# NilFoundation/crypto3-zk

Measured on AMD Instinct MI355X. Metric: MSM Mpoints/sec, BLS12-381 G1 Pippenger, 2^20 points per GPU, higher is better.
Workload: dtype u32; 1 GPU; BLS12-381 G1 Pippenger MSM, ONE MSM of 1 x 2^20 random points/scalars, bases resident; points_per_gpu=1048576, parallelism=point-range partition x1 + one all-gather of the 144-B partial sums

## Files before the change

### crypto3-zk_amd/csrc/arith_ops.h

```cpp
#pragma once
#include "curve.hpp"
#include "fu_safegcd.hpp"

namespace zkhip {
namespace arith {

template <class U>
struct MaxSpread {
    static constexpr int K = 128;
};
template <>
struct MaxSpread<BlsFrU> {
    static constexpr int K = 64;
};
template <>
struct MaxSpread<PallasFrU> {
    static constexpr int K = 64;
};
template <>
struct MaxSpread<VestaFrU> {
    static constexpr int K = 64;
};

template <class U>
ZK_HD bool fu_raw_valid(int op) {
    if (op >= 0 && op <= 10) return true;
    return op >= 21 && op <= 27 && (1 << (op - 20)) <= MaxSpread<U>::K;
}

template <int K, class U>
ZK_HD Fu<U> sub_k(const Fu<U> &a, const Fu<U> &b) {
    if constexpr (K <= MaxSpread<U>::K) return fu_sub<K>(a, b);
    return Fu<U>::zero();
}

template <class U>
ZK_HD void fu_raw_one(int op, const uint32_t *a, const uint32_t *b, const uint32_t *c, const uint32_t *d, uint32_t *out) {
    constexpr int L = U::L;
    Fu<U> x, y, z, w, r = Fu<U>::zero();
    for (int i = 0; i < L; ++i) x.v[i] = a[i], y.v[i] = b[i], z.v[i] = c[i], w.v[i] = d[i];
    switch (op) {
        case 0: r = fu_mul(x, y); break;
        case 1: r = fu_sqr(x); break;
        case 2: r = fu_mul2(x, y, z, w); break;
        case 3: r = fu_add(x, y); break;
        case 4: r = fu_cond_sub_p(x); break;
        case 5: r = fu_canon(x); break;
        case 6: r.v[0] = fu_is_zero_lt2p(x) ? 1u : 0u; break;
        case 7: r = fu_inv(x); break;
        case 8: r = fu_inv_gcd(x); break;
        case 9: {
            uint32_t s[U::NL];
            fu_pack<U>(s, x);
            for (int i = 0; i < U::NL; ++i) r.v[i] = s[i];
            break;
        }
        case 10: r = fu_unpack<U>(a); break;
        case 21: r = sub_k<2>(x, y); break;
        case 22: r = sub_k<4>(x, y); break;
        case 23: r = sub_k<8>(x, y); break;
        case 24: r = sub_k<16>(x, y); break;
        case 25: r = sub_k<32>(x, y); break;
        case 26: r = sub_k<64>(x, y); break;
        case 27: r = sub_k<128>(x, y); break;
        default: break;
    }
    for (int i = 0; i < L; ++i) out[i] = r.v[i];
}

template <class F>
ZK_HD F sqr_direct(const F &x) { return FieldOps<F>::sqr(x); }
template <class U>
ZK_HD Fu<U> sqr_direct(const Fu<U> &x) { return fu_sqr(x); }

template <class F>
ZK_HD F inv_gcd(const F &x) { return FieldOps<F>::inv(x); }
template <class U>
ZK_HD Fu<U> inv_gcd(const Fu<U> &x) { return fu_inv_gcd(fu_canon(x)); }

ZK_HD bool field_op_valid(int op) { return op >= 0 && op <= 11; }

template <class F>
ZK_HD void field_op(int op, const uint32_t *a, const uint32_t *b, uint32_t *out) {
    typedef FieldOps<F> O;
    F x = O::from_canonical(a), y = b ? O::from_canonical(b) : F::zero(), r = F::zero();
    switch (op) {
        case 0: r = O::mul(x, y); break;
        case 1: r = O::add(x, y); break;
        case 2: r = O::template sub<O::K1>(x, y); break;
        case 3: r = O::inv(x); break;
// ... 1 lines not shown
        case 5: r = O::template sub<O::K1>(F::zero(), x); break;
        case 6: r = O::add(x, x); break;
        case 7: r = O::template sub<O::K2>(x, y); break;
        case 9: r = sqr_direct(O::add(x, y)); break;
        case 10: r = O::template mul_sub<O::K2>(x, O::add(x, y), O::template sub<O::K1>(F::zero(), y), y); break;
        case 11: r = inv_gcd(x); break;
        case 8: {
            F ab = O::mul(x, y), bb = O::sqr(y);
            F X = O::template sub<O::K1>(O::sqr(x), O::add(ab, O::add(bb, bb)));
            r = O::mul(O::template sub<O::K2>(ab, X), O::template sub<O::K2>(bb, X));
            break;
        }
        default: break;
    }
    O::to_canonical(out, r);
}

template <class F>
ZK_HD Affine<F> load_aff(const uint32_t *p, int inf) {
    typedef FieldOps<F> O;
    if (inf) return Affine<F>::infinity();
    return {O::from_canonical(p), O::from_canonical(p + O::CANON_WORDS)};
}
template <class F>
ZK_HD void store_aff(uint32_t *p, uint8_t *inf, const XYZZ<F> &a) {
    typedef FieldOps<F> O;
    Affine<F> r = xyzz_to_affine(a);
    *inf = a.is_inf() ? 1 : 0;
    O::to_canonical(p, r.x);
    O::to_canonical(p + O::CANON_WORDS, r.y);
}

template <class F>
ZK_HD void point_chain(const uint32_t *pts, const uint8_t *inf, const uint8_t *neg, size_t n, int mode, uint32_t k, uint32_t *out,
                       uint8_t *out_inf) {
    typedef FieldOps<F> O;
    constexpr int CW = O::CANON_WORDS;
    size_t split = mode == 1 ? n / 2 : n;
    XYZZ<F> acc = XYZZ<F>::infinity(), acc2 = XYZZ<F>::infinity();
    alignas(16) uint32_t b16[4 * O::WORDS];
    for (size_t i = 0; i < split; ++i) {
        Affine<F> p = load_aff<F>(pts + i * 2 * CW, inf ? inf[i] : 0);
        if (mode == 4) {
            affine_store<F>(b16, p);
            p = affine_load<F>(b16);
        }
        acc = xyzz_madd(acc, p, neg ? neg[i] != 0 : false);
        if (mode == 4) {
            xyzz_store<F>(b16, acc);
            acc = xyzz_load<F>(b16);
        }
    }
    for (size_t i = split; i < n; ++i) acc2 = xyzz_madd(acc2, load_aff<F>(pts + i * 2 * CW, inf ? inf[i] : 0), neg ? neg[i] != 0 : false);
    if (mode == 1) acc = xyzz_add(acc, acc2);
    if (mode == 2) acc = xyzz_mul_small(acc, k);
    if (mode == 3) {
        Jacobian<F> j = xyzz_to_jacobian(acc);
        O::to_canonical(out, j.X);
        O::to_canonical(out + CW, j.Y);
        O::to_canonical(out + 2 * CW, j.Z);
        *out_inf = acc.is_inf() ? 1 : 0;
        return;
    }
    store_aff<F>(out, out_inf, acc);
}

}
}
```

### crypto3-zk_amd/csrc/curve.hpp

```cpp
#pragma once
#include "fu.hpp"

namespace zkhip {

template <class F>
struct Affine {
    F x, y;
    ZK_HD bool is_inf() const { return FieldOps<F>::is_exact_zero(x) && FieldOps<F>::is_exact_zero(y); }
    ZK_HD static Affine infinity() { return {F::zero(), F::zero()}; }
};

template <class F>
struct XYZZ {
    F X, Y, ZZ, ZZZ;
    ZK_HD bool is_inf() const { return FieldOps<F>::is_exact_zero(ZZ); }
    ZK_HD static XYZZ infinity() { return {F::zero(), F::zero(), F::zero(), F::zero()}; }
    ZK_HD static XYZZ from_affine(const Affine<F> &p) {
        if (p.is_inf()) return infinity();
        return {p.x, p.y, F::one(), F::one()};
    }
};

template <class F>
struct Jacobian {
    F X, Y, Z;
};

template <class F>
ZK_HD XYZZ<F> xyzz_dbl_affine(const Affine<F> &p) {
    typedef FieldOps<F> O;
    if (p.is_inf()) return XYZZ<F>::infinity();
    F U = O::add(p.y, p.y);
    F V = O::sqr(U);
    F W = O::mul(U, V);
    F S = O::mul(p.x, V);
    F xx = O::sqr(p.x);
    F M = O::add(O::add(xx, xx), xx);
    F X3 = O::template sub<O::K1>(O::sqr(M), O::add(S, S));
    F Y3 = O::template mul_sub<O::K2>(M, O::template sub<O::K2>(S, X3), W, p.y);
    return {X3, Y3, V, W};
}

template <class F>
ZK_HD XYZZ<F> xyzz_dbl(const XYZZ<F> &a) {
    typedef FieldOps<F> O;
    if (a.is_inf()) return XYZZ<F>::infinity();
    F U = O::add(a.Y, a.Y);
    F V = O::sqr(U);
    F W = O::mul(U, V);
    F S = O::mul(a.X, V);
    F xx = O::sqr(a.X);
    F M = O::add(O::add(xx, xx), xx);
    F X3 = O::template sub<O::K1>(O::sqr(M), O::add(S, S));
    F Y3 = O::template mul_sub<O::K2>(M, O::template sub<O::K2>(S, X3), W, a.Y);
    return {X3, Y3, O::mul(V, a.ZZ), O::mul(W, a.ZZZ)};
}

template <class F>
ZK_HD XYZZ<F> xyzz_madd(const XYZZ<F> &a, const Affine<F> &p_in, bool negate = false) {
    typedef FieldOps<F> O;
    if (p_in.is_inf()) return a;
    Affine<F> p = p_in;
    if (negate) p.y = O::template sub<O::K1>(F::zero(), p.y);
    if (a.is_inf()) return {p.x, p.y, F::one(), F::one()};
    F U2 = O::mul(p.x, a.ZZ);
    F S2 = O::mul(p.y, a.ZZZ);
    F Pd = O::template sub<O::K2>(U2, a.X);
    F R = O::template sub<O::K2>(S2, a.Y);
    F PP = O::sqr(Pd);
    if (O::is_zero_product(PP)) {
        if (O::is_zero(R)) return xyzz_dbl_affine(p);
        return XYZZ<F>::infinity();
    }
    F PPP = O::mul(Pd, PP);
    F Q = O::mul(a.X, PP);
    F X3 = O::template sub<O::K1>(O::sqr(R), O::add(PPP, O::add(Q, Q)));
    F Y3 = O::template mul_sub<O::K2>(R, O::template sub<O::K2>(Q, X3), a.Y, PPP);
    return {X3, Y3, O::mul(a.ZZ, PP), O::mul(a.ZZZ, PPP)};
}

template <class F>
ZK_HD XYZZ<F> xyzz_add(const XYZZ<F> &a, const XYZZ<F> &b) {
    typedef FieldOps<F> O;
    if (a.is_inf()) return b;
    if (b.is_inf()) return a;
    F U1 = O::mul(a.X, b.ZZ);
    F U2 = O::mul(b.X, a.ZZ);
    F S1 = O::mul(a.Y, b.ZZZ);
    F S2 = O::mul(b.Y, a.ZZZ);
    F Pd = O::template sub<O::K1>(U2, U1);
    F R = O::template sub<O::K1>(S2, S1);
    F PP = O::sqr(Pd);
    if (O::is_zero_product(PP)) {
        if (O::is_zero(R)) return xyzz_dbl(a);
        return XYZZ<F>::infinity();
    }
    F PPP = O::mul(Pd, PP);
    F Q = O::mul(U1, PP);
    F X3 = O::template sub<O::K1>(O::sqr(R), O::add(PPP, O::add(Q, Q)));
    F Y3 = O::template mul_sub<O::K1>(R, O::template sub<O::K2>(Q, X3), S1, PPP);
    return {X3, Y3, O::mul(O::mul(a.ZZ, b.ZZ), PP), O::mul(O::mul(a.ZZZ, b.ZZZ), PPP)};
}

template <class F>
ZK_HD XYZZ<F> xyzz_mul_small(const XYZZ<F> &a, uint32_t k) {
    XYZZ<F> r = XYZZ<F>::infinity();
    if (k == 0 || a.is_inf()) return r;
    int top = 31;
    while (!((k >> top) & 1)) --top;
    if (top == 0) return a;
    const XYZZ<F> a2 = xyzz_dbl(a), a3 = xyzz_add(a2, a);
    for (int i = top >> 1; i >= 0; --i) {
        if (!r.is_inf()) r = xyzz_dbl(xyzz_dbl(r));
        const uint32_t d = (k >> (2 * i)) & 3u;
        if (d != 0) r = xyzz_add(r, d == 1 ? a : (d == 2 ? a2 : a3));
    }
    return r;
}

template <class F>
ZK_HD Jacobian<F> xyzz_to_jacobian(const XYZZ<F> &a) {
    typedef FieldOps<F> O;
    if (a.is_inf()) return {F::one(), F::one(), F::zero()};
    F z2 = O::sqr(a.ZZ);
    F z3 = O::sqr(a.ZZZ);
    return {O::mul(a.X, O::sqr(z2)), O::mul(a.Y, O::sqr(z3)), O::mul(a.ZZ, a.ZZZ)};
}

template <class F>
ZK_HD XYZZ<F> xyzz_from_jacobian(const Jacobian<F> &j) {
    typedef FieldOps<F> O;
    if (O::is_zero(j.Z)) return XYZZ<F>::infinity();
// ... 68 lines not shown
```

### crypto3-zk_amd/csrc/fu.hpp

```cpp
#pragma once
#include "fp.hpp"
#if defined(__HIP_DEVICE_COMPILE__) && !defined(ZK_NO_ASM_MUL)
#define ZK_ASM_MUL 1
#include "mont_asm.hpp"
#endif

namespace zkhip {

template <class U>
struct Fu {
    typedef U params;
    static constexpr int L = U::L;
    static constexpr int B = U::B;
    static constexpr int SL = U::SL;
    static constexpr uint32_t MASK = (1u << U::B) - 1;
    uint32_t v[L];

    ZK_HD static Fu zero() {
        Fu r;
ZK_UNROLL
        for (int i = 0; i < L; ++i) r.v[i] = 0;
        return r;
    }
    ZK_HD static Fu one() {
// ... 13 lines not shown
ZK_UNROLL
        for (int i = 0; i < L; ++i) r.v[i] = U::mod(i);
        return r;
    }
    ZK_HD bool limbs_zero() const {
        uint32_t o = 0;
ZK_UNROLL
        for (int i = 0; i < L; ++i) o |= v[i];
        return o == 0;
    }
    ZK_HD bool limbs_equal(const Fu &b) const {
        uint32_t o = 0;
ZK_UNROLL
        for (int i = 0; i < L; ++i) o |= v[i] ^ b.v[i];
        return o == 0;
    }
};

template <class U>
ZK_HD void fu_norm(Fu<U> &a) {
    constexpr int L = U::L, B = U::B;
ZK_UNROLL
    for (int i = 0; i < L - 1; ++i) {
        a.v[i + 1] += a.v[i] >> B;
        a.v[i] &= Fu<U>::MASK;
    }
}

template <class U>
ZK_HD Fu<U> fu_add(const Fu<U> &a, const Fu<U> &b) {
    Fu<U> r;
ZK_UNROLL
    for (int i = 0; i < U::L; ++i) r.v[i] = a.v[i] + b.v[i];
    fu_norm(r);
    return r;
}

template <int K, class U>
ZK_HD Fu<U> fu_sub(const Fu<U> &a, const Fu<U> &b) {
    Fu<U> r;
ZK_UNROLL
    for (int i = 0; i < U::L; ++i) r.v[i] = a.v[i] + (U::template spread<K>(i) - b.v[i]);
    fu_norm(r);
    return r;
}

template <class U>
ZK_HD Fu<U> fu_mul(const Fu<U> &a, const Fu<U> &b) {
    constexpr int L = U::L, B = U::B;
    constexpr uint32_t MASK = Fu<U>::MASK;
    Fu<U> r;
#ifdef ZK_ASM_MUL
    static_assert(B == 29, "mont_asm.hpp is generated for 29-bit limbs");
    uint32_t p[L];
ZK_UNROLL
    for (int i = 0; i < L; ++i) p[i] = U::mod(i);
    MontAsm<L>::mul(r.v, a.v, b.v, p, U::QINV);
    return r;
#endif
    uint32_t m[L];
    uint64_t acc = 0;
ZK_UNROLL
    for (int k = 0; k < L; ++k) {
ZK_UNROLL
        for (int i = 0; i <= k; ++i) acc += (uint64_t)a.v[i] * b.v[k - i];
ZK_UNROLL
// ... 209 lines not shown
        uint4 t;
        t.x = 4 * i + 0 < L ? a.v[4 * i + 0] : 0u;
        t.y = 4 * i + 1 < L ? a.v[4 * i + 1] : 0u;
        t.z = 4 * i + 2 < L ? a.v[4 * i + 2] : 0u;
        t.w = 4 * i + 3 < L ? a.v[4 * i + 3] : 0u;
        q[i] = t;
    }
}

template <class U>
struct Fu2 {
    typedef U params;
    Fu<U> c0, c1;
    ZK_HD static Fu2 zero() { return {Fu<U>::zero(), Fu<U>::zero()}; }
    ZK_HD static Fu2 one() { return {Fu<U>::one(), Fu<U>::zero()}; }
    ZK_HD bool limbs_zero() const { return c0.limbs_zero() && c1.limbs_zero(); }
};

template <class F>
struct FieldOps;

template <class P>
struct FieldOps<Fp<P>> {
    typedef Fp<P> F;
    static constexpr int K1 = 2, K2 = 2, K3 = 2;
    static constexpr int WORDS = P::NL;
    ZK_HD static F mul(const F &a, const F &b) { return a * b; }
    ZK_HD static F sqr(const F &a) { return a * a; }
    ZK_HD static F add(const F &a, const F &b) { return a + b; }
    template <int K>
    ZK_HD static F sub(const F &a, const F &b) { return a - b; }
    template <int K>
    ZK_HD static F mul_sub(const F &a, const F &b, const F &c, const F &d) { return mul(a, b) - mul(c, d); }
    ZK_HD static bool is_zero(const F &a) { return a.is_zero(); }
    ZK_HD static bool is_zero_product(const F &a) { return a.is_zero(); }
    ZK_HD static bool is_exact_zero(const F &a) { return a.is_zero(); }
    ZK_HD static F load(const uint32_t *p) { return fp_load<P>(p); }
    ZK_HD static void store(uint32_t *p, const F &a) { fp_store<P>(p, a); }
    ZK_HD static F from_canonical(const uint32_t *sat) { return fp_to_mont(fp_load<P>(sat)); }
    ZK_HD static void to_canonical(uint32_t *sat, const F &a) { fp_store<P>(sat, fp_from_mont(a)); }
    static constexpr int CANON_WORDS = P::NL;
    ZK_HD static F inv(const F &a) { return fp_inv(a); }
};

template <class P>
struct FieldOps<Fp2<P>> {
    typedef Fp2<P> F;
    static constexpr int K1 = 2, K2 = 2, K3 = 2;
    static constexpr int WORDS = 2 * P::NL;
    ZK_HD static F mul(const F &a, const F &b) { return a * b; }
    ZK_HD static F sqr(const F &a) { return fp_sqr(a); }
    ZK_HD static F add(const F &a, const F &b) { return a + b; }
    template <int K>
    ZK_HD static F sub(const F &a, const F &b) { return a - b; }
    template <int K>
    ZK_HD static F mul_sub(const F &a, const F &b, const F &c, const F &d) { return mul(a, b) - mul(c, d); }
    ZK_HD static bool is_zero(const F &a) { return a.is_zero(); }
    ZK_HD static bool is_zero_product(const F &a) { return a.is_zero(); }
    ZK_HD static bool is_exact_zero(const F &a) { return a.is_zero(); }
    ZK_HD static F load(const uint32_t *p) { return {fp_load<P>(p), fp_load<P>(p + P::NL)}; }
    ZK_HD static void store(uint32_t *p, const F &a) {
        fp_store<P>(p, a.c0);
        fp_store<P>(p + P::NL, a.c1);
    }
    ZK_HD static F from_canonical(const uint32_t *sat) { return {fp_to_mont(fp_load<P>(sat)), fp_to_mont(fp_load<P>(sat + P::NL))}; }
    ZK_HD static void to_canonical(uint32_t *sat, const F &a) {
        fp_store<P>(sat, fp_from_mont(a.c0));
        fp_store<P>(sat + P::NL, fp_from_mont(a.c1));
    }
    static constexpr int CANON_WORDS = 2 * P::NL;
    ZK_HD static F inv(const F &a) { return fp_inv(a); }
};

template <class U>
ZK_HD Fu<U> fu_mul_sel(const Fu<U> &a, const Fu<U> &b) {
#ifdef ZK_NOINLINE_MUL
    return fu_mul_call(a, b);
#else
    return fu_mul(a, b);
#endif
}

template <class U>
ZK_HD Fu<U> fu_mul_sel2(const Fu<U> &a, const Fu<U> &b) {
#if defined(ZK_NOINLINE_MUL) || defined(ZK_NOINLINE_MUL2)
    return fu_mul_call(a, b);
#else
    return fu_mul(a, b);
#endif
// ... 20 lines not shown
    }
    const Fu<U> a2 = fu_mul_call(a, a), a3 = fu_mul_call(a2, a);
    Fu<U> r = Fu<U>::one();
    for (int i = NL * 32 - 2; i >= 0; i -= 2) {
        r = fu_sqr_call(fu_sqr_call(r));
        const uint32_t w = (e[i >> 5] >> (i & 31)) & 3u;
        if (w == 1) r = fu_mul_call(r, a);
        else if (w == 2) r = fu_mul_call(r, a2);
        else if (w == 3) r = fu_mul_call(r, a3);
    }
    return r;
}

template <class U>
struct FieldOps<Fu<U>> {
    typedef Fu<U> F;
    static constexpr int K1 = 8, K2 = 16, K3 = 32;
    static constexpr int WORDS = U::SL;
    ZK_HD static F mul(const F &a, const F &b) { return fu_mul_sel(a, b); }
    ZK_HD static F sqr(const F &a) {
#ifdef ZK_NOINLINE_MUL
        return fu_mul_call(a, a);
#else
        return fu_sqr(a);
#endif
    }
    ZK_HD static F add(const F &a, const F &b) { return fu_add(a, b); }
    template <int K>
    ZK_HD static F sub(const F &a, const F &b) { return fu_sub<K>(a, b); }
    template <int K>
    ZK_HD static F mul_sub(const F &a, const F &b, const F &c, const F &d) {
        return fu_mul2_sel(a, b, fu_sub<K>(F::zero(), c), d);
    }
    ZK_HD static bool is_zero(const F &a) { return fu_canon(a).limbs_zero(); }
    ZK_HD static bool is_zero_product(const F &a) { return fu_is_zero_lt2p(a); }
    ZK_HD static bool is_exact_zero(const F &a) { return a.limbs_zero(); }
    ZK_HD static F load(const uint32_t *p) { return fu_load<U>(p); }
    ZK_HD static void store(uint32_t *p, const F &a) { fu_store<U>(p, a); }
    ZK_HD static F from_canonical(const uint32_t *sat) { return fu_from_canonical<U>(sat); }
    ZK_HD static void to_canonical(uint32_t *sat, const F &a) { fu_to_canonical<U>(sat, a); }
    static constexpr int CANON_WORDS = U::NL;
    ZK_HD static F inv(const F &a) { return fu_inv(a); }
};

template <class U>
struct FieldOps<Fu2<U>> {
    typedef Fu2<U> F;
    typedef FieldOps<Fu<U>> B;
    static constexpr int K1 = 32, K2 = 64, K3 = 128;
    static constexpr int WORDS = 2 * U::SL;
    ZK_HD static F mul(const F &a, const F &b) {
        Fu<U> v0 = fu_mul_sel2(a.c0, b.c0), v1 = fu_mul_sel2(a.c1, b.c1);
        Fu<U> s = fu_mul_sel2(fu_add(a.c0, a.c1), fu_add(b.c0, b.c1));
        return {fu_sub<4>(v0, v1), fu_sub<8>(s, fu_add(v0, v1))};
    }
    ZK_HD static F sqr(const F &a) {
        Fu<U> t = fu_mul_sel2(fu_add(a.c0, a.c1), fu_sub<128>(a.c0, a.c1));
        Fu<U> m = fu_mul_sel2(a.c0, a.c1);
        return {t, fu_add(m, m)};
    }
    ZK_HD static F add(const F &a, const F &b) { return {fu_add(a.c0, b.c0), fu_add(a.c1, b.c1)}; }
    template <int K>
    ZK_HD static F sub(const F &a, const F &b) { return {fu_sub<K>(a.c0, b.c0), fu_sub<K>(a.c1, b.c1)}; }
    template <int K>
    ZK_HD static F mul_sub(const F &a, const F &b, const F &c, const F &d) { return sub<K1>(mul(a, b), mul(c, d)); }
    ZK_HD static bool is_zero(const F &a) { return fu_canon(a.c0).limbs_zero() && fu_canon(a.c1).limbs_zero(); }
    ZK_HD static bool is_zero_product(const F &a) { return is_zero(a); }
    ZK_HD static bool is_exact_zero(const F &a) { return a.limbs_zero(); }
    ZK_HD static F load(const uint32_t *p) { return {fu_load<U>(p), fu_load<U>(p + U::SL)}; }
    ZK_HD static void store(uint32_t *p, const F &a) {
        fu_store<U>(p, a.c0);
        fu_store<U>(p + U::SL, a.c1);
    }
    ZK_HD static F from_canonical(const uint32_t *sat) { return {fu_from_canonical<U>(sat), fu_from_canonical<U>(sat + U::NL)}; }
    ZK_HD static void to_canonical(uint32_t *sat, const F &a) {
        fu_to_canonical<U>(sat, a.c0);
        fu_to_canonical<U>(sat + U::NL, a.c1);
    }
    static constexpr int CANON_WORDS = 2 * U::NL;
    ZK_HD static F inv(const F &a) {
        Fu<U> n = fu_inv(fu_add(fu_mul_sel2(a.c0, a.c0), fu_mul_sel2(a.c1, a.c1)));
        return {fu_mul_sel2(a.c0, n), fu_sub<4>(Fu<U>::zero(), fu_mul_sel2(a.c1, n))};
    }
};

typedef Fu<BlsFqU> bls_fqu;
typedef Fu<BnFqU> bn_fqu;
typedef Fu<BlsFrU> bls_fru;
typedef Fu<BnFrU> bn_fru;
typedef Fu<PallasFqU> pallas_fqu;
typedef Fu<VestaFqU> vesta_fqu;
typedef Fu<PallasFrU> pallas_fru;
typedef Fu<VestaFrU> vesta_fru;
typedef Fu2<BlsFqU> bls_fqu2;
typedef Fu2<BnFqU> bn_fqu2;

template <class T>
struct FieldTag { typedef T type; };
// ... 20 lines not shown
```

### crypto3-zk_amd/csrc/fu2_pair.hpp

```cpp
#pragma once
#include "curve.hpp"

namespace zkhip {

template <class U>
struct Fu2h {
    typedef U params;
    Fu<U> v;
    ZK_D static bool odd() { return (threadIdx.x & 1u) != 0; }
    ZK_D static Fu2h zero() { return {Fu<U>::zero()}; }
    ZK_D static Fu2h one() { return {odd() ? Fu<U>::zero() : Fu<U>::one()}; }
};

ZK_D uint32_t pair_swap(uint32_t x) { return (uint32_t)__builtin_amdgcn_update_dpp(0, (int)x, 0xB1 , 0xF, 0xF, false); }
template <class U>
ZK_D Fu<U> pair_swap(const Fu<U> &a) {
    Fu<U> r;
#pragma unroll
    for (int i = 0; i < U::L; ++i) r.v[i] = pair_swap(a.v[i]);
    return r;
}
template <class U>
ZK_D Fu<U> fu_select(bool c, const Fu<U> &a, const Fu<U> &b) {
    Fu<U> r;
// ... 15 lines not shown
    const Fu<U> ao = pair_swap(a);
    return fu_mul(fu_add(a, fu_select(odd, a, ao)), fu_select(odd, ao, fu_sub<128>(a, ao)));
}

template <class U>
struct FieldOps<Fu2h<U>> {
    typedef Fu2h<U> F;
    static constexpr int K1 = 16, K2 = 32, K3 = 64;
    static constexpr int WORDS = 2 * U::SL;
    ZK_D static F mul(const F &a, const F &b) {
#ifdef ZK_PAIR_INLINE
        const bool odd = F::odd();
        const Fu<U> ao = pair_swap(a.v), bo = pair_swap(b.v);
        const Fu<U> x2 = fu_select(odd, ao, fu_sub<128>(Fu<U>::zero(), ao));
        return {fu_mul2(a.v, fu_select(odd, bo, b.v), x2, fu_select(odd, b.v, bo))};
#else
        return {fu2h_mul_call(a.v, b.v)};
#endif
    }
    ZK_D static F sqr(const F &a) {
#ifdef ZK_PAIR_INLINE
        const bool odd = F::odd();
        const Fu<U> ao = pair_swap(a.v);
        return {fu_mul(fu_add(a.v, fu_select(odd, a.v, ao)), fu_select(odd, ao, fu_sub<128>(a.v, ao)))};
#else
        return {fu2h_sqr_call(a.v)};
#endif
    }
    ZK_D static F add(const F &a, const F &b) { return {fu_add(a.v, b.v)}; }
    template <int K>
    ZK_D static F sub(const F &a, const F &b) { return {fu_sub<K>(a.v, b.v)}; }
    template <int K>
    ZK_D static F mul_sub(const F &a, const F &b, const F &c, const F &d) { return sub<K1>(mul(a, b), mul(c, d)); }
    ZK_D static bool both(bool mine) {
        const uint32_t m = mine ? 1u : 0u, o = pair_swap(m);
        return (m & o) != 0;
    }
    ZK_D static bool is_zero(const F &a) { return both(fu_canon(a.v).limbs_zero()); }
    ZK_D static bool is_zero_product(const F &a) { return both(fu_is_zero_lt2p(a.v)); }
    ZK_D static bool is_exact_zero(const F &a) { return both(a.v.limbs_zero()); }
    static constexpr int CANON_WORDS = 2 * U::NL;
    ZK_D static void to_canonical(uint32_t *sat, const F &a) { fu_to_canonical<U>(sat + (F::odd() ? U::NL : 0), a.v); }
    ZK_D static F load(const uint32_t *p) { return {fu_load<U>(p + (F::odd() ? U::SL : 0))}; }
    ZK_D static void store(uint32_t *p, const F &a) { fu_store<U>(p + (F::odd() ? U::SL : 0), a.v); }
};

template <class F>
struct BucketLane {
    typedef F type;
    static constexpr int LANES = 1;
};
template <class U>
struct BucketLane<Fu2<U>> {
    typedef Fu2h<U> type;
    static constexpr int LANES = 2;
};

}
```

### crypto3-zk_amd/csrc/fu_pair.hpp

```cpp
#pragma once
#include "curve.hpp"
#include "fu2_pair.hpp"

namespace zkhip {

template <class U>
struct FuP {
    typedef U params;
    Fu<U> v;
    ZK_D static bool odd() { return (threadIdx.x & 1u) != 0; }
    ZK_D static FuP zero() { return {Fu<U>::zero()}; }
    ZK_D static FuP one() { return {Fu<U>::one()}; }
};

template <class U>
struct FieldOps<FuP<U>> {
    typedef FuP<U> F;
    typedef FieldOps<Fu<U>> B;
    static constexpr int K1 = B::K1, K2 = B::K2, K3 = B::K3;
    static constexpr int WORDS = U::SL;
    static constexpr int CANON_WORDS = U::NL;
    ZK_D static F mul(const F &a, const F &b) { return {fu_mul_call(a.v, b.v)}; }
    ZK_D static F sqr(const F &a) { return {fu_mul_call(a.v, a.v)}; }
    ZK_D static F add(const F &a, const F &b) { return {fu_add(a.v, b.v)}; }
    template <int K>
    ZK_D static F sub(const F &a, const F &b) { return {fu_sub<K>(a.v, b.v)}; }
    template <int K>
    ZK_D static F mul_sub(const F &a, const F &b, const F &c, const F &d) { return {fu_mul2_call(a.v, b.v, fu_sub<K>(Fu<U>::zero(), c.v), d.v)}; }
    ZK_D static bool is_zero(const F &a) { return fu_canon(a.v).limbs_zero(); }
    ZK_D static bool is_zero_product(const F &a) { return fu_is_zero_lt2p(a.v); }
    ZK_D static bool is_exact_zero(const F &a) { return a.v.limbs_zero(); }
    ZK_D static F load(const uint32_t *p) { return {fu_load<U>(p)}; }
    ZK_D static void store(uint32_t *p, const F &a) { fu_store<U>(p, a.v); }
    ZK_D static void to_canonical(uint32_t *sat, const F &a) { fu_to_canonical<U>(sat, a.v); }
};

template <class U>
struct PairProducts {
    Fu<U> even, odd;
};
template <class U>
ZK_D PairProducts<U> pair_mul(const Fu<U> &ae, const Fu<U> &be, const Fu<U> &ao, const Fu<U> &bo) {
    const bool odd = FuP<U>::odd();
    const Fu<U> mine = fu_mul(fu_select(odd, ao, ae), fu_select(odd, bo, be));
    const Fu<U> other = pair_swap(mine);
    return {fu_select(odd, other, mine), fu_select(odd, mine, other)};
}
template <class U>
ZK_D PairProducts<U> pair_sqr(const Fu<U> &ae, const Fu<U> &ao) {
    const bool odd = FuP<U>::odd();
    const Fu<U> mine = fu_sqr(fu_select(odd, ao, ae));
    const Fu<U> other = pair_swap(mine);
    return {fu_select(odd, other, mine), fu_select(odd, mine, other)};
}
template <class U>
ZK_D PairProducts<U> pair_mul2_mul(const Fu<U> &ae, const Fu<U> &be, const Fu<U> &ce, const Fu<U> &de, const Fu<U> &ao, const Fu<U> &bo) {
    const bool odd = FuP<U>::odd();
    const Fu<U> z = Fu<U>::zero();
    const Fu<U> mine = fu_mul2(fu_select(odd, ao, ae), fu_select(odd, bo, be), fu_select(odd, z, ce), fu_select(odd, z, de));
    const Fu<U> other = pair_swap(mine);
    return {fu_select(odd, other, mine), fu_select(odd, mine, other)};
}

template <class U>
ZK_D XYZZ<FuP<U>> xyzz_dbl(const XYZZ<FuP<U>> &a) {
    typedef FieldOps<Fu<U>> O;
    if (a.is_inf()) return XYZZ<FuP<U>>::infinity();
    const Fu<U> Uu = fu_add(a.Y.v, a.Y.v);
    const PairProducts<U> s1 = pair_sqr(Uu, a.X.v);
    const Fu<U> &V = s1.even, &XX = s1.odd;
    const PairProducts<U> s2 = pair_mul(Uu, V, a.X.v, V);
    const Fu<U> &W = s2.even, &S = s2.odd;
    const Fu<U> M = fu_add(fu_add(XX, XX), XX);
    const PairProducts<U> s3 = pair_mul(M, M, V, a.ZZ.v);
    const Fu<U> X3 = fu_sub<O::K1>(s3.even, fu_add(S, S));
    const PairProducts<U> s4 = pair_mul2_mul(M, fu_sub<O::K2>(S, X3), fu_sub<O::K2>(Fu<U>::zero(), W), a.Y.v, W, a.ZZZ.v);
    return {{X3}, {s4.even}, {s3.odd}, {s4.odd}};
}

template <class U>
ZK_D XYZZ<FuP<U>> xyzz_add(const XYZZ<FuP<U>> &a, const XYZZ<FuP<U>> &b) {
    typedef FieldOps<Fu<U>> O;
    if (a.is_inf()) return b;
    if (b.is_inf()) return a;
    const PairProducts<U> s1 = pair_mul(a.X.v, b.ZZ.v, b.X.v, a.ZZ.v);
    const PairProducts<U> s2 = pair_mul(a.Y.v, b.ZZZ.v, b.Y.v, a.ZZZ.v);
    const Fu<U> &U1 = s1.even, &S1 = s2.even;
    const Fu<U> Pd = fu_sub<O::K1>(s1.odd, U1), R = fu_sub<O::K1>(s2.odd, S1);
    const PairProducts<U> s3 = pair_sqr(Pd, R);
    const Fu<U> &PP = s3.even;
    if (fu_is_zero_lt2p(PP)) {
        if (fu_canon(R).limbs_zero()) return xyzz_dbl(a);
        return XYZZ<FuP<U>>::infinity();
    }
    const PairProducts<U> s4 = pair_mul(Pd, PP, U1, PP);
    const Fu<U> &PPP = s4.even, &Q = s4.odd;
    const Fu<U> X3 = fu_sub<O::K1>(s3.odd, fu_add(PPP, fu_add(Q, Q)));
    const PairProducts<U> s5 = pair_mul2_mul(R, fu_sub<O::K2>(Q, X3), fu_sub<O::K1>(Fu<U>::zero(), S1), PPP, a.ZZ.v, b.ZZ.v);
    const PairProducts<U> s6 = pair_mul(a.ZZZ.v, b.ZZZ.v, s5.odd, PP);
    const PairProducts<U> s7 = pair_mul(s6.even, PPP, s6.even, PPP);
    return {{X3}, {s5.even}, {s6.odd}, {s7.even}};
}

template <class U>
ZK_D XYZZ<FuP<U>> xyzz_mul_small(const XYZZ<FuP<U>> &a, uint32_t k) {
    XYZZ<FuP<U>> r = XYZZ<FuP<U>>::infinity();
    if (k == 0 || a.is_inf()) return r;
    int top = 31;
    while (!((k >> top) & 1)) --top;
    r = a;
    for (int i = top - 1; i >= 0; --i) {
        r = xyzz_dbl(r);
        if ((k >> i) & 1) r = xyzz_add(r, a);
    }
    return r;
}

template <class F>
struct TailLane : BucketLane<F> { };
template <class U>
struct TailLane<Fu<U>> {
    typedef FuP<U> type;
    static constexpr int LANES = 2;
};

}
```

### crypto3-zk_amd/csrc/fu_quad.hpp

```cpp
#pragma once
#include "fu_pair.hpp"

namespace zkhip {

template <class U>
struct FuQ {
    typedef U params;
    Fu<U> v;
    ZK_D static uint32_t lane() { return threadIdx.x & 3u; }
    ZK_D static FuQ zero() { return {Fu<U>::zero()}; }
    ZK_D static FuQ one() { return {Fu<U>::one()}; }
};

template <class U>
struct FieldOps<FuQ<U>> {
    typedef FuQ<U> F;
    typedef FieldOps<Fu<U>> B;
    static constexpr int K1 = B::K1, K2 = B::K2, K3 = B::K3;
    static constexpr int WORDS = U::SL;
    static constexpr int CANON_WORDS = U::NL;
    ZK_D static F mul(const F &a, const F &b) { return {fu_mul_call(a.v, b.v)}; }
    ZK_D static F sqr(const F &a) { return {fu_mul_call(a.v, a.v)}; }
    ZK_D static F add(const F &a, const F &b) { return {fu_add(a.v, b.v)}; }
    template <int K>
    ZK_D static F sub(const F &a, const F &b) { return {fu_sub<K>(a.v, b.v)}; }
    template <int K>
    ZK_D static F mul_sub(const F &a, const F &b, const F &c, const F &d) { return {fu_mul2_call(a.v, b.v, fu_sub<K>(Fu<U>::zero(), c.v), d.v)}; }
    ZK_D static bool is_zero(const F &a) { return fu_canon(a.v).limbs_zero(); }
    ZK_D static bool is_zero_product(const F &a) { return fu_is_zero_lt2p(a.v); }
    ZK_D static bool is_exact_zero(const F &a) { return a.v.limbs_zero(); }
    ZK_D static F load(const uint32_t *p) { return {fu_load<U>(p)}; }
    ZK_D static void store(uint32_t *p, const F &a) { fu_store<U>(p, a.v); }
    ZK_D static void to_canonical(uint32_t *sat, const F &a) { fu_to_canonical<U>(sat, a.v); }
};

template <int K>
ZK_D uint32_t quad_bcast(uint32_t x) {
    uint32_t r = (uint32_t)__builtin_amdgcn_update_dpp(0, (int)x, K * 0x55 , 0xF, 0xF, false);
    asm volatile("" : "+v"(r));
    return r;
}
template <int K, class U>
ZK_D Fu<U> quad_bcast(const Fu<U> &a) {
    Fu<U> r;
#pragma unroll
    for (int i = 0; i < U::L; ++i) r.v[i] = quad_bcast<K>(a.v[i]);
    return r;
}
template <class U>
ZK_D Fu<U> quad_select(uint32_t lane, const Fu<U> &a0, const Fu<U> &a1, const Fu<U> &a2, const Fu<U> &a3) {
    const bool b0 = (lane & 1u) != 0, b1 = (lane & 2u) != 0;
    return fu_select(b1, fu_select(b0, a3, a2), fu_select(b0, a1, a0));
}

template <class U>
struct QuadProducts {
    Fu<U> p0, p1, p2, p3;
};
template <class U>
ZK_D QuadProducts<U> quad_mul(const Fu<U> &a0, const Fu<U> &b0, const Fu<U> &a1, const Fu<U> &b1, const Fu<U> &a2, const Fu<U> &b2, const Fu<U> &a3,
                              const Fu<U> &b3) {
    const uint32_t lane = FuQ<U>::lane();
    const Fu<U> mine = fu_mul(quad_select(lane, a0, a1, a2, a3), quad_select(lane, b0, b1, b2, b3));
    return {quad_bcast<0>(mine), quad_bcast<1>(mine), quad_bcast<2>(mine), quad_bcast<3>(mine)};
}

template <class U>
ZK_D XYZZ<FuQ<U>> xyzz_dbl(const XYZZ<FuQ<U>> &a) {
    typedef FieldOps<Fu<U>> O;
    if (a.is_inf()) return XYZZ<FuQ<U>>::infinity();
    const Fu<U> Uu = fu_add(a.Y.v, a.Y.v);
    const QuadProducts<U> s1 = quad_mul(Uu, Uu, a.X.v, a.X.v, Uu, Uu, a.X.v, a.X.v);
    const Fu<U> &V = s1.p0, &XX = s1.p1;
    const Fu<U> M = fu_add(fu_add(XX, XX), XX);
    const QuadProducts<U> s2 = quad_mul(Uu, V, a.X.v, V, V, a.ZZ.v, M, M);
    const Fu<U> &W = s2.p0, &S = s2.p1;
    const Fu<U> X3 = fu_sub<O::K1>(s2.p3, fu_add(S, S));
    const Fu<U> D = fu_sub<O::K2>(S, X3);
    const QuadProducts<U> s3 = quad_mul(M, D, W, a.Y.v, W, a.ZZZ.v, M, D);
    return {{X3}, {fu_sub<O::K1>(s3.p0, s3.p1)}, {s2.p2}, {s3.p2}};
}

template <class U>
ZK_D XYZZ<FuQ<U>> xyzz_add(const XYZZ<FuQ<U>> &a, const XYZZ<FuQ<U>> &b) {
    typedef FieldOps<Fu<U>> O;
    if (a.is_inf()) return b;
    if (b.is_inf()) return a;
    const QuadProducts<U> s1 = quad_mul(a.X.v, b.ZZ.v, b.X.v, a.ZZ.v, a.Y.v, b.ZZZ.v, b.Y.v, a.ZZZ.v);
    const Fu<U> &U1 = s1.p0, &S1 = s1.p2;
    const Fu<U> Pd = fu_sub<O::K1>(s1.p1, U1), R = fu_sub<O::K1>(s1.p3, S1);
    const QuadProducts<U> s2 = quad_mul(Pd, Pd, R, R, a.ZZ.v, b.ZZ.v, a.ZZZ.v, b.ZZZ.v);
    const Fu<U> &PP = s2.p0;
    if (fu_is_zero_lt2p(PP)) {
        if (fu_canon(R).limbs_zero()) return xyzz_dbl(a);
        return XYZZ<FuQ<U>>::infinity();
    }
    const QuadProducts<U> s3 = quad_mul(Pd, PP, U1, PP, s2.p2, PP, Pd, PP);
    const Fu<U> &PPP = s3.p0, &Q = s3.p1;
    const Fu<U> X3 = fu_sub<O::K1>(s2.p1, fu_add(PPP, fu_add(Q, Q)));
    const Fu<U> D = fu_sub<O::K2>(Q, X3);
    const QuadProducts<U> s4 = quad_mul(R, D, S1, PPP, s2.p3, PPP, R, D);
    return {{X3}, {fu_sub<O::K1>(s4.p0, s4.p1)}, {s3.p2}, {s4.p2}};
}

template <class U>
ZK_D XYZZ<FuQ<U>> xyzz_mul_small(const XYZZ<FuQ<U>> &a, uint32_t k) {
    XYZZ<FuQ<U>> r = XYZZ<FuQ<U>>::infinity();
    if (k == 0 || a.is_inf()) return r;
    int top = 31;
    while (!((k >> top) & 1)) --top;
    r = a;
    for (int i = top - 1; i >= 0; --i) {
        r = xyzz_dbl(r);
        if ((k >> i) & 1) r = xyzz_add(r, a);
    }
    return r;
}

template <class F>
struct QuadLane {
    static constexpr bool AVAILABLE = false;
    typedef typename TailLane<F>::type type;
    static constexpr int LANES = TailLane<F>::LANES;
};
template <class U>
struct QuadLane<Fu<U>> {
    static constexpr bool AVAILABLE = true;
    typedef FuQ<U> type;
    static constexpr int LANES = 4;
};

}
// ... 1 lines not shown
```

### crypto3-zk_amd/csrc/msm_bucket_acc.hpp

```cpp
#pragma once
#include "curve.hpp"
#include "fu2_pair.hpp"

namespace zkhip {

template <class F>
struct LimbView;
template <class U>
struct LimbView<Fu<U>> {
    static constexpr int N = U::L;
    ZK_D static uint32_t get(const Fu<U> &x, int i) { return x.v[i]; }
    ZK_D static void set(Fu<U> &x, int i, uint32_t v) { x.v[i] = v; }
};
template <class U>
struct LimbView<Fu2h<U>> {
    static constexpr int N = U::L;
    ZK_D static uint32_t get(const Fu2h<U> &x, int i) { return x.v.v[i]; }
    ZK_D static void set(Fu2h<U> &x, int i, uint32_t v) { x.v.v[i] = v; }
};

template <class F, int NT>
struct LdsAcc {
    typedef LimbView<F> V;
    static constexpr int Q = (V::N + 3) / 4;
// ... 8 lines not shown
            w[4 * q] = v.x, w[4 * q + 1] = v.y, w[4 * q + 2] = v.z, w[4 * q + 3] = v.w;
        }
        F r;
#pragma unroll
        for (int i = 0; i < V::N; ++i) V::set(r, i, w[i]);
        return r;
    }
    ZK_D void put(int coord, const F &x) const {
#pragma unroll
        for (int q = 0; q < Q; ++q) {
            uint4 v;
            v.x = 4 * q + 0 < V::N ? V::get(x, 4 * q + 0) : 0u;
            v.y = 4 * q + 1 < V::N ? V::get(x, 4 * q + 1) : 0u;
            v.z = 4 * q + 2 < V::N ? V::get(x, 4 * q + 2) : 0u;
            v.w = 4 * q + 3 < V::N ? V::get(x, 4 * q + 3) : 0u;
            base[(coord * Q + q) * NT + t] = v;
        }
    }
};

template <class F, int NT, int WAVES, int LPB = 1>
__global__ __launch_bounds__(NT, WAVES) void msm_bucket_acc_lds(const uint32_t *__restrict__ bases, const uint32_t *__restrict__ offs,
                                                           const uint32_t *__restrict__ idx, uint32_t nbuckets, uint32_t large,
                                                           const uint32_t *__restrict__ order, uint32_t *__restrict__ buckets) {
    typedef FieldOps<F> O;
    constexpr int NL = O::WORDS;
    extern __shared__ __attribute__((aligned(16))) uint4 acc_lds[];
    const uint32_t tid = threadIdx.x, slot = (blockIdx.x * NT + tid) / LPB;
    if (slot >= nbuckets) return;
    const uint32_t g = order[slot];
    const uint32_t lo = offs[g], hi = offs[g + 1];
    if (hi - lo > large) return;
    LdsAcc<F, NT> A = {acc_lds, tid};
    enum { CX = 0, CY = 1, CZZ = 2 };
    F ZZZ = F::zero();
    bool inf = true;
    for (uint32_t k = lo; k < hi; ++k) {
        const uint32_t e = idx[k];
        Affine<F> p = affine_load<F>(bases + (size_t)(e & 0x7FFFFFFFu) * (2 * NL));
        if (p.is_inf()) continue;
        if (e >> 31) p.y = O::template sub<O::K1>(F::zero(), p.y);
        if (inf) {
            A.put(CX, p.x);
            A.put(CY, p.y);
            A.put(CZZ, F::one());
            ZZZ = F::one();
            inf = false;
            continue;
        }
        F Pd = O::template sub<O::K2>(O::mul(p.x, A.get(CZZ)), A.get(CX));
        F R = O::template sub<O::K2>(O::mul(p.y, ZZZ), A.get(CY));
        F PP = O::sqr(Pd);
        if (O::is_zero_product(PP)) {
            if (O::is_zero(R)) {
                XYZZ<F> d = xyzz_dbl_affine(p);
                A.put(CX, d.X);
                A.put(CY, d.Y);
                A.put(CZZ, d.ZZ);
                ZZZ = d.ZZZ;
            } else {
                inf = true;
            }
            continue;
        }
        F PPP = O::mul(Pd, PP);
        F Q = O::mul(A.get(CX), PP);
        F X3 = O::template sub<O::K1>(O::sqr(R), O::add(PPP, O::add(Q, Q)));
        F Y3 = O::template mul_sub<O::K2>(R, O::template sub<O::K2>(Q, X3), A.get(CY), PPP);
        A.put(CX, X3);
        A.put(CY, Y3);
        A.put(CZZ, O::mul(A.get(CZZ), PP));
        ZZZ = O::mul(ZZZ, PPP);
    }
    XYZZ<F> out = XYZZ<F>::infinity();
    if (!inf) out = {A.get(CX), A.get(CY), A.get(CZZ), ZZZ};
    xyzz_store<F>(buckets + (size_t)g * (4 * NL), out);
}

}
```

Measured before the change: 397.9 Mpoints/s.

## Track affine bucket state and sign-flip Y to skip muls in bucket accumulation

Bucket accumulation now keeps a state word that distinguishes empty, affine and XYZZ buckets. For the second point it does a cheap affine+affine add with no ZZ/ZZZ multiplies. It stores Y with an alternating sign so the Y3 update uses mul_add instead of negate plus mul_sub, and adds a three-operand add3 that fuses chained additions with a single normalisation. This trims field multiplies and normalisations in the hot loop, at the cost of extra state branches and a final conditional negation; new test ops and modes expose the helpers.

```diff
diff --git a/crypto3-zk_amd/csrc/arith_ops.h b/crypto3-zk_amd/csrc/arith_ops.h
--- a/crypto3-zk_amd/csrc/arith_ops.h
+++ b/crypto3-zk_amd/csrc/arith_ops.h
@@ -24,7 +24,7 @@
 
 template <class U>
 ZK_HD bool fu_raw_valid(int op) {
-    if (op >= 0 && op <= 10) return true;
+    if ((op >= 0 && op <= 10) || op == 12 || op == 13) return true;
     return op >= 21 && op <= 27 && (1 << (op - 20)) <= MaxSpread<U>::K;
 }
 
@@ -56,6 +56,8 @@
             break;
         }
         case 10: r = fu_unpack<U>(a); break;
+        case 12: r = fu_add3(x, y, z); break;
+        case 13: r = fu_mul2(x, fu_sub<8>(y, w), z, w); break;
         case 21: r = sub_k<2>(x, y); break;
         case 22: r = sub_k<4>(x, y); break;
         case 23: r = sub_k<8>(x, y); break;
@@ -123,6 +125,13 @@
 }
 
 template <class F>
+struct PlainAcc {
+    F c[3];
+    ZK_HD F get(int coord) const { return c[coord]; }
+    ZK_HD void put(int coord, const F &x) { c[coord] = x; }
+};
+
+template <class F>
 ZK_HD void point_chain(const uint32_t *pts, const uint8_t *inf, const uint8_t *neg, size_t n, int mode, uint32_t k, uint32_t *out,
                        uint8_t *out_inf) {
     typedef FieldOps<F> O;
@@ -130,6 +139,25 @@
     size_t split = mode == 1 ? n / 2 : n;
     XYZZ<F> acc = XYZZ<F>::infinity(), acc2 = XYZZ<F>::infinity();
     alignas(16) uint32_t b16[4 * O::WORDS];
+    if (mode == 6) {
+        PlainAcc<F> A = {{F::zero(), F::zero(), F::zero()}};
+        F ZZZ = F::zero();
+        uint32_t st = BKT_EMPTY;
+        for (size_t i = 0; i < n; ++i) bucket_step(A, ZZZ, st, load_aff<F>(pts + i * 2 * CW, inf ? inf[i] : 0), neg ? neg[i] != 0 : false);
+        store_aff<F>(out, out_inf, bucket_finish(A, ZZZ, st));
+        return;
+    }
+    if (mode == 7) {
+        Affine<F> q[2] = {Affine<F>::infinity(), Affine<F>::infinity()};
+        for (size_t i = 0; i < n && i < 2; ++i) {
+            q[i] = load_aff<F>(pts + i * 2 * CW, inf ? inf[i] : 0);
+            if (neg && neg[i] && !q[i].is_inf()) q[i].y = O::template sub<O::K1>(F::zero(), q[i].y);
+        }
+        acc = xyzz_add_affine(q[0], q[1]);
+        for (size_t i = 2; i < n; ++i) acc = xyzz_madd(acc, load_aff<F>(pts + i * 2 * CW, inf ? inf[i] : 0), neg ? neg[i] != 0 : false);
+        store_aff<F>(out, out_inf, acc);
+        return;
+    }
     for (size_t i = 0; i < split; ++i) {
         Affine<F> p = load_aff<F>(pts + i * 2 * CW, inf ? inf[i] : 0);
         if (mode == 4) {
diff --git a/crypto3-zk_amd/csrc/curve.hpp b/crypto3-zk_amd/csrc/curve.hpp
--- a/crypto3-zk_amd/csrc/curve.hpp
+++ b/crypto3-zk_amd/csrc/curve.hpp
@@ -35,7 +35,7 @@
     F W = O::mul(U, V);
     F S = O::mul(p.x, V);
     F xx = O::sqr(p.x);
-    F M = O::add(O::add(xx, xx), xx);
+    F M = O::add3(xx, xx, xx);
     F X3 = O::template sub<O::K1>(O::sqr(M), O::add(S, S));
     F Y3 = O::template mul_sub<O::K2>(M, O::template sub<O::K2>(S, X3), W, p.y);
     return {X3, Y3, V, W};
@@ -50,7 +50,7 @@
     F W = O::mul(U, V);
     F S = O::mul(a.X, V);
     F xx = O::sqr(a.X);
-    F M = O::add(O::add(xx, xx), xx);
+    F M = O::add3(xx, xx, xx);
     F X3 = O::template sub<O::K1>(O::sqr(M), O::add(S, S));
     F Y3 = O::template mul_sub<O::K2>(M, O::template sub<O::K2>(S, X3), W, a.Y);
     return {X3, Y3, O::mul(V, a.ZZ), O::mul(W, a.ZZZ)};
@@ -74,9 +74,91 @@
     }
     F PPP = O::mul(Pd, PP);
     F Q = O::mul(a.X, PP);
-    F X3 = O::template sub<O::K1>(O::sqr(R), O::add(PPP, O::add(Q, Q)));
+    F X3 = O::template sub<O::K1>(O::sqr(R), O::add3(PPP, Q, Q));
     F Y3 = O::template mul_sub<O::K2>(R, O::template sub<O::K2>(Q, X3), a.Y, PPP);
     return {X3, Y3, O::mul(a.ZZ, PP), O::mul(a.ZZZ, PPP)};
+}
+
+template <class F>
+ZK_HD XYZZ<F> xyzz_add_affine(const Affine<F> &p1, const Affine<F> &p2) {
+    typedef FieldOps<F> O;
+    if (p1.is_inf()) return XYZZ<F>::from_affine(p2);
+    if (p2.is_inf()) return XYZZ<F>::from_affine(p1);
+    F Pd = O::template sub<O::K2>(p2.x, p1.x);
+    F R = O::template sub<O::K2>(p2.y, p1.y);
+    F PP = O::sqr(Pd);
+    if (O::is_zero_product(PP)) {
+        if (O::is_zero(R)) return xyzz_dbl_affine(p1);
+        return XYZZ<F>::infinity();
+    }
+    F PPP = O::mul(Pd, PP);
+    F Q = O::mul(p1.x, PP);
+    F X3 = O::template sub<O::K1>(O::sqr(R), O::add3(PPP, Q, Q));
+    F Y3 = O::template mul_sub<O::K2>(R, O::template sub<O::K2>(Q, X3), p1.y, PPP);
+    return {X3, Y3, PP, PPP};
+}
+
+enum { ACC_X = 0, ACC_W = 1, ACC_ZZ = 2 };
+enum : uint32_t { BKT_EMPTY = 0, BKT_AFFINE = 1, BKT_XYZZ = 2, BKT_KIND = 3, BKT_MINUS = 4  };
+
+template <class F, class Acc>
+ZK_HD void bucket_step(Acc &A, F &ZZZ, uint32_t &st, Affine<F> p, bool negate) {
+    typedef FieldOps<F> O;
+    if (p.is_inf()) return;
+    if (negate != ((st & BKT_MINUS) != 0)) p.y = O::template sub<O::K1>(F::zero(), p.y);
+    if ((st & BKT_KIND) == BKT_EMPTY) {
+        A.put(ACC_X, p.x);
+        A.put(ACC_W, p.y);
+        A.put(ACC_ZZ, F::one());
+        ZZZ = F::one();
+        st = BKT_AFFINE;
+        return;
+    }
+    const bool affine = (st & BKT_KIND) == BKT_AFFINE;
+    F U2 = p.x, S2 = p.y;
+    if (!affine) {
+        U2 = O::mul(p.x, A.get(ACC_ZZ));
+        S2 = O::mul(p.y, ZZZ);
+    }
+    F Pd = O::template sub<O::K2>(U2, A.get(ACC_X));
+    F Rt = O::template sub<O::K2>(S2, A.get(ACC_W));
+    F PP = O::sqr(Pd);
+    if (O::is_zero_product(PP)) {
+        if (O::is_zero(Rt)) {
+            XYZZ<F> d = xyzz_dbl_affine(p);
+            A.put(ACC_X, d.X);
+            A.put(ACC_W, d.Y);
+            A.put(ACC_ZZ, d.ZZ);
+            ZZZ = d.ZZZ;
+            st = BKT_XYZZ | (st & BKT_MINUS);
+        } else {
+            st = BKT_EMPTY;
+        }
+        return;
+    }
+    F PPP = O::mul(Pd, PP);
+    F Q = O::mul(A.get(ACC_X), PP);
+    F X3 = O::template sub<O::K1>(O::sqr(Rt), O::add3(PPP, Q, Q));
+    F W3 = O::mul_add(Rt, O::template sub<O::K1>(X3, Q), A.get(ACC_W), PPP);
+    A.put(ACC_X, X3);
+    A.put(ACC_W, W3);
+    if (affine) {
+        A.put(ACC_ZZ, PP);
+        ZZZ = PPP;
+    } else {
+        A.put(ACC_ZZ, O::mul(A.get(ACC_ZZ), PP));
+        ZZZ = O::mul(ZZZ, PPP);
+    }
+    st = BKT_XYZZ | (~st & BKT_MINUS);
+}
+
+template <class F, class Acc>
+ZK_HD XYZZ<F> bucket_finish(const Acc &A, const F &ZZZ, uint32_t st) {
+    typedef FieldOps<F> O;
+    if ((st & BKT_KIND) == BKT_EMPTY) return XYZZ<F>::infinity();
+    F Y = A.get(ACC_W);
+    if (st & BKT_MINUS) Y = O::template sub<O::KW>(F::zero(), Y);
+    return {A.get(ACC_X), Y, A.get(ACC_ZZ), ZZZ};
 }
 
 template <class F>
@@ -97,7 +179,7 @@
     }
     F PPP = O::mul(Pd, PP);
     F Q = O::mul(U1, PP);
-    F X3 = O::template sub<O::K1>(O::sqr(R), O::add(PPP, O::add(Q, Q)));
+    F X3 = O::template sub<O::K1>(O::sqr(R), O::add3(PPP, Q, Q));
     F Y3 = O::template mul_sub<O::K1>(R, O::template sub<O::K2>(Q, X3), S1, PPP);
     return {X3, Y3, O::mul(O::mul(a.ZZ, b.ZZ), PP), O::mul(O::mul(a.ZZZ, b.ZZZ), PPP)};
 }
diff --git a/crypto3-zk_amd/csrc/fu.hpp b/crypto3-zk_amd/csrc/fu.hpp
--- a/crypto3-zk_amd/csrc/fu.hpp
+++ b/crypto3-zk_amd/csrc/fu.hpp
@@ -69,6 +69,15 @@
     Fu<U> r;
 ZK_UNROLL
     for (int i = 0; i < U::L; ++i) r.v[i] = a.v[i] + b.v[i];
+    fu_norm(r);
+    return r;
+}
+
+template <class U>
+ZK_HD Fu<U> fu_add3(const Fu<U> &a, const Fu<U> &b, const Fu<U> &c) {
+    Fu<U> r;
+ZK_UNROLL
+    for (int i = 0; i < U::L; ++i) r.v[i] = a.v[i] + b.v[i] + c.v[i];
     fu_norm(r);
     return r;
 }
@@ -344,6 +353,9 @@
     ZK_HD static F sub(const F &a, const F &b) { return a - b; }
     template <int K>
     ZK_HD static F mul_sub(const F &a, const F &b, const F &c, const F &d) { return mul(a, b) - mul(c, d); }
+    static constexpr int KW = 2;
+    ZK_HD static F add3(const F &a, const F &b, const F &c) { return a + b + c; }
+    ZK_HD static F mul_add(const F &a, const F &b, const F &c, const F &d) { return mul(a, b) + mul(c, d); }
     ZK_HD static bool is_zero(const F &a) { return a.is_zero(); }
     ZK_HD static bool is_zero_product(const F &a) { return a.is_zero(); }
     ZK_HD static bool is_exact_zero(const F &a) { return a.is_zero(); }
@@ -367,6 +379,9 @@
     ZK_HD static F sub(const F &a, const F &b) { return a - b; }
     template <int K>
     ZK_HD static F mul_sub(const F &a, const F &b, const F &c, const F &d) { return mul(a, b) - mul(c, d); }
+    static constexpr int KW = 2;
+    ZK_HD static F add3(const F &a, const F &b, const F &c) { return a + b + c; }
+    ZK_HD static F mul_add(const F &a, const F &b, const F &c, const F &d) { return mul(a, b) + mul(c, d); }
     ZK_HD static bool is_zero(const F &a) { return a.is_zero(); }
     ZK_HD static bool is_zero_product(const F &a) { return a.is_zero(); }
     ZK_HD static bool is_exact_zero(const F &a) { return a.is_zero(); }
@@ -453,6 +468,9 @@
     ZK_HD static F mul_sub(const F &a, const F &b, const F &c, const F &d) {
         return fu_mul2_sel(a, b, fu_sub<K>(F::zero(), c), d);
     }
+    static constexpr int KW = K1;
+    ZK_HD static F add3(const F &a, const F &b, const F &c) { return fu_add3(a, b, c); }
+    ZK_HD static F mul_add(const F &a, const F &b, const F &c, const F &d) { return fu_mul2_sel(a, b, c, d); }
     ZK_HD static bool is_zero(const F &a) { return fu_canon(a).limbs_zero(); }
     ZK_HD static bool is_zero_product(const F &a) { return fu_is_zero_lt2p(a); }
     ZK_HD static bool is_exact_zero(const F &a) { return a.limbs_zero(); }
@@ -485,6 +503,9 @@
     ZK_HD static F sub(const F &a, const F &b) { return {fu_sub<K>(a.c0, b.c0), fu_sub<K>(a.c1, b.c1)}; }
     template <int K>
     ZK_HD static F mul_sub(const F &a, const F &b, const F &c, const F &d) { return sub<K1>(mul(a, b), mul(c, d)); }
+    static constexpr int KW = K2;
+    ZK_HD static F add3(const F &a, const F &b, const F &c) { return {fu_add3(a.c0, b.c0, c.c0), fu_add3(a.c1, b.c1, c.c1)}; }
+    ZK_HD static F mul_add(const F &a, const F &b, const F &c, const F &d) { return add(mul(a, b), mul(c, d)); }
     ZK_HD static bool is_zero(const F &a) { return fu_canon(a.c0).limbs_zero() && fu_canon(a.c1).limbs_zero(); }
     ZK_HD static bool is_zero_product(const F &a) { return is_zero(a); }
     ZK_HD static bool is_exact_zero(const F &a) { return a.limbs_zero(); }
diff --git a/crypto3-zk_amd/csrc/fu2_pair.hpp b/crypto3-zk_amd/csrc/fu2_pair.hpp
--- a/crypto3-zk_amd/csrc/fu2_pair.hpp
+++ b/crypto3-zk_amd/csrc/fu2_pair.hpp
@@ -71,6 +71,9 @@
     ZK_D static F sub(const F &a, const F &b) { return {fu_sub<K>(a.v, b.v)}; }
     template <int K>
     ZK_D static F mul_sub(const F &a, const F &b, const F &c, const F &d) { return sub<K1>(mul(a, b), mul(c, d)); }
+    static constexpr int KW = K2;
+    ZK_D static F add3(const F &a, const F &b, const F &c) { return {fu_add3(a.v, b.v, c.v)}; }
+    ZK_D static F mul_add(const F &a, const F &b, const F &c, const F &d) { return add(mul(a, b), mul(c, d)); }
     ZK_D static bool both(bool mine) {
         const uint32_t m = mine ? 1u : 0u, o = pair_swap(m);
         return (m & o) != 0;
diff --git a/crypto3-zk_amd/csrc/fu_pair.hpp b/crypto3-zk_amd/csrc/fu_pair.hpp
--- a/crypto3-zk_amd/csrc/fu_pair.hpp
+++ b/crypto3-zk_amd/csrc/fu_pair.hpp
@@ -27,6 +27,9 @@
     ZK_D static F sub(const F &a, const F &b) { return {fu_sub<K>(a.v, b.v)}; }
     template <int K>
     ZK_D static F mul_sub(const F &a, const F &b, const F &c, const F &d) { return {fu_mul2_call(a.v, b.v, fu_sub<K>(Fu<U>::zero(), c.v), d.v)}; }
+    static constexpr int KW = K1;
+    ZK_D static F add3(const F &a, const F &b, const F &c) { return {fu_add3(a.v, b.v, c.v)}; }
+    ZK_D static F mul_add(const F &a, const F &b, const F &c, const F &d) { return {fu_mul2_call(a.v, b.v, c.v, d.v)}; }
     ZK_D static bool is_zero(const F &a) { return fu_canon(a.v).limbs_zero(); }
     ZK_D static bool is_zero_product(const F &a) { return fu_is_zero_lt2p(a.v); }
     ZK_D static bool is_exact_zero(const F &a) { return a.v.limbs_zero(); }
@@ -71,7 +74,7 @@
     const Fu<U> &V = s1.even, &XX = s1.odd;
     const PairProducts<U> s2 = pair_mul(Uu, V, a.X.v, V);
     const Fu<U> &W = s2.even, &S = s2.odd;
-    const Fu<U> M = fu_add(fu_add(XX, XX), XX);
+    const Fu<U> M = fu_add3(XX, XX, XX);
     const PairProducts<U> s3 = pair_mul(M, M, V, a.ZZ.v);
     const Fu<U> X3 = fu_sub<O::K1>(s3.even, fu_add(S, S));
     const PairProducts<U> s4 = pair_mul2_mul(M, fu_sub<O::K2>(S, X3), fu_sub<O::K2>(Fu<U>::zero(), W), a.Y.v, W, a.ZZZ.v);
@@ -95,7 +98,7 @@
     }
     const PairProducts<U> s4 = pair_mul(Pd, PP, U1, PP);
     const Fu<U> &PPP = s4.even, &Q = s4.odd;
-    const Fu<U> X3 = fu_sub<O::K1>(s3.odd, fu_add(PPP, fu_add(Q, Q)));
+    const Fu<U> X3 = fu_sub<O::K1>(s3.odd, fu_add3(PPP, Q, Q));
     const PairProducts<U> s5 = pair_mul2_mul(R, fu_sub<O::K2>(Q, X3), fu_sub<O::K1>(Fu<U>::zero(), S1), PPP, a.ZZ.v, b.ZZ.v);
     const PairProducts<U> s6 = pair_mul(a.ZZZ.v, b.ZZZ.v, s5.odd, PP);
     const PairProducts<U> s7 = pair_mul(s6.even, PPP, s6.even, PPP);
diff --git a/crypto3-zk_amd/csrc/fu_quad.hpp b/crypto3-zk_amd/csrc/fu_quad.hpp
--- a/crypto3-zk_amd/csrc/fu_quad.hpp
+++ b/crypto3-zk_amd/csrc/fu_quad.hpp
@@ -26,6 +26,9 @@
     ZK_D static F sub(const F &a, const F &b) { return {fu_sub<K>(a.v, b.v)}; }
     template <int K>
     ZK_D static F mul_sub(const F &a, const F &b, const F &c, const F &d) { return {fu_mul2_call(a.v, b.v, fu_sub<K>(Fu<U>::zero(), c.v), d.v)}; }
+    static constexpr int KW = K1;
+    ZK_D static F add3(const F &a, const F &b, const F &c) { return {fu_add3(a.v, b.v, c.v)}; }
+    ZK_D static F mul_add(const F &a, const F &b, const F &c, const F &d) { return {fu_mul2_call(a.v, b.v, c.v, d.v)}; }
     ZK_D static bool is_zero(const F &a) { return fu_canon(a.v).limbs_zero(); }
     ZK_D static bool is_zero_product(const F &a) { return fu_is_zero_lt2p(a.v); }
     ZK_D static bool is_exact_zero(const F &a) { return a.v.limbs_zero(); }
@@ -72,7 +75,7 @@
     const Fu<U> Uu = fu_add(a.Y.v, a.Y.v);
     const QuadProducts<U> s1 = quad_mul(Uu, Uu, a.X.v, a.X.v, Uu, Uu, a.X.v, a.X.v);
     const Fu<U> &V = s1.p0, &XX = s1.p1;
-    const Fu<U> M = fu_add(fu_add(XX, XX), XX);
+    const Fu<U> M = fu_add3(XX, XX, XX);
     const QuadProducts<U> s2 = quad_mul(Uu, V, a.X.v, V, V, a.ZZ.v, M, M);
     const Fu<U> &W = s2.p0, &S = s2.p1;
     const Fu<U> X3 = fu_sub<O::K1>(s2.p3, fu_add(S, S));
@@ -97,7 +100,7 @@
     }
     const QuadProducts<U> s3 = quad_mul(Pd, PP, U1, PP, s2.p2, PP, Pd, PP);
     const Fu<U> &PPP = s3.p0, &Q = s3.p1;
-    const Fu<U> X3 = fu_sub<O::K1>(s2.p1, fu_add(PPP, fu_add(Q, Q)));
+    const Fu<U> X3 = fu_sub<O::K1>(s2.p1, fu_add3(PPP, Q, Q));
     const Fu<U> D = fu_sub<O::K2>(Q, X3);
     const QuadProducts<U> s4 = quad_mul(R, D, S1, PPP, s2.p3, PPP, R, D);
     return {{X3}, {fu_sub<O::K1>(s4.p0, s4.p1)}, {s3.p2}, {s4.p2}};
diff --git a/crypto3-zk_amd/csrc/msm_bucket_acc.hpp b/crypto3-zk_amd/csrc/msm_bucket_acc.hpp
--- a/crypto3-zk_amd/csrc/msm_bucket_acc.hpp
+++ b/crypto3-zk_amd/csrc/msm_bucket_acc.hpp
@@ -64,49 +64,14 @@
     const uint32_t lo = offs[g], hi = offs[g + 1];
     if (hi - lo > large) return;
     LdsAcc<F, NT> A = {acc_lds, tid};
-    enum { CX = 0, CY = 1, CZZ = 2 };
     F ZZZ = F::zero();
-    bool inf = true;
+    uint32_t st = BKT_EMPTY;
     for (uint32_t k = lo; k < hi; ++k) {
         const uint32_t e = idx[k];
-        Affine<F> p = affine_load<F>(bases + (size_t)(e & 0x7FFFFFFFu) * (2 * NL));
-        if (p.is_inf()) continue;
-        if (e >> 31) p.y = O::template sub<O::K1>(F::zero(), p.y);
-        if (inf) {
-            A.put(CX, p.x);
-            A.put(CY, p.y);
-            A.put(CZZ, F::one());
-            ZZZ = F::one();
-            inf = false;
-            continue;
-        }
-        F Pd = O::template sub<O::K2>(O::mul(p.x, A.get(CZZ)), A.get(CX));
-        F R = O::template sub<O::K2>(O::mul(p.y, ZZZ), A.get(CY));
-        F PP = O::sqr(Pd);
-        if (O::is_zero_product(PP)) {
-            if (O::is_zero(R)) {
-                XYZZ<F> d = xyzz_dbl_affine(p);
-                A.put(CX, d.X);
-                A.put(CY, d.Y);
-                A.put(CZZ, d.ZZ);
-                ZZZ = d.ZZZ;
-            } else {
-                inf = true;
-            }
-            continue;
-        }
-        F PPP = O::mul(Pd, PP);
-        F Q = O::mul(A.get(CX), PP);
-        F X3 = O::template sub<O::K1>(O::sqr(R), O::add(PPP, O::add(Q, Q)));
-        F Y3 = O::template mul_sub<O::K2>(R, O::template sub<O::K2>(Q, X3), A.get(CY), PPP);
-        A.put(CX, X3);
-        A.put(CY, Y3);
-        A.put(CZZ, O::mul(A.get(CZZ), PP));
-        ZZZ = O::mul(ZZZ, PPP);
+        const Affine<F> p = affine_load<F>(bases + (size_t)(e & 0x7FFFFFFFu) * (2 * NL));
+        bucket_step(A, ZZZ, st, p, (e >> 31) != 0);
     }
-    XYZZ<F> out = XYZZ<F>::infinity();
-    if (!inf) out = {A.get(CX), A.get(CY), A.get(CZZ), ZZZ};
-    xyzz_store<F>(buckets + (size_t)g * (4 * NL), out);
+    xyzz_store<F>(buckets + (size_t)g * (4 * NL), bucket_finish(A, ZZZ, st));
 }
 
 }
```

After: 411.1 Mpoints/s, median of 6. +3.3%, better.
